# dpfried/action-segmentation

Hardware: AMD Instinct MI355X
Metric: frames/sec semi-Markov decode, CrossTask T~10k K~20 L=1024, 1/2/4/8 GPUs (higher is better)
Workload: dtype f64

## Files before the change

### action-segmentation_amd/csrc/smm_api.hip

```cpp
#include <algorithm>
#include <atomic>
#include <functional>
#include <cstdio>
#include <cstdlib>
#include <cstring>
#include <numeric>
#include <vector>
#include <unordered_map>
#include <mutex>
#include <utility>
#include <string>

#include "../../include/smmdp.h"
#include "smm_device.h"
#include "smm_launch.h"
#include "smm_plan_feedback.h"

static thread_local int g_last_hip = 0;

namespace {
struct SmmEnv {
    int spec = 1;
    int no_split = 0;
    double split_min_us = 100.0, split_ns = 0.0;
    int split_margin = 400;
    int plan_cache = 1;
    int small_wg = 1;
    int plan_feedback = 1;
    int chunk = 1;
    int chunk_p = 0;
    int chunk_lmin = 0;
    int chunk_wc = 512;
    int no_bt_window = 0;
    int fit_grid = 0;
    int verbose = 0;
#ifdef SMM_DEV
    int debug_flags = 0;
    int split_debug = 0;
    int upload_memcpy = 0;
    int emission_v2 = 0;
#endif
    std::string key;
};
std::atomic<const SmmEnv *> g_env{nullptr};
std::once_flag g_env_once;

void env_read()
{
    SmmEnv e;
    struct Item { const char *name; int *i; double *d; };
    const Item items[] = {
        {"SMM_SPEC", &e.spec, nullptr}, {"SMM_NO_SPLIT", &e.no_split, nullptr}, {"SMM_SPLIT_MIN_US", nullptr, &e.split_min_us},
        {"SMM_SPLIT_NS", nullptr, &e.split_ns}, {"SMM_SPLIT_MARGIN", &e.split_margin, nullptr},
        {"SMM_PLAN_CACHE", &e.plan_cache, nullptr}, {"SMM_SMALL_WG", &e.small_wg, nullptr}, {"SMM_PLAN_FEEDBACK", &e.plan_feedback, nullptr}, {"SMM_CHUNK", &e.chunk, nullptr}, {"SMM_CHUNK_P", &e.chunk_p, nullptr},
        {"SMM_CHUNK_WC", &e.chunk_wc, nullptr}, {"SMM_CHUNK_LMIN", &e.chunk_lmin, nullptr}, {"SMM_NO_BT_WINDOW", &e.no_bt_window, nullptr},
        {"SMM_FIT_GRID", &e.fit_grid, nullptr}, {"SMM_VERBOSE", &e.verbose, nullptr},
#ifdef SMM_DEV
        {"SMM_DEBUG_FLAGS", &e.debug_flags, nullptr}, {"SMM_SPLIT_DEBUG", &e.split_debug, nullptr},
        {"SMM_UPLOAD_MEMCPY", &e.upload_memcpy, nullptr}, {"SMM_EMISSION_V2", &e.emission_v2, nullptr},
#endif
    };
    for (const Item &it : items) {
        const char *v = std::getenv(it.name);
        if (!v) continue;
        if (it.i) *it.i = (*v == 0) ? 1 : std::atoi(v);
        if (it.d) *it.d = std::atof(v);
        e.key += it.name; e.key += '='; e.key += v; e.key += ';';
    }
    g_env.store(new SmmEnv(e), std::memory_order_release);
}
const SmmEnv &env()
{
    std::call_once(g_env_once, env_read);
    return *g_env.load(std::memory_order_acquire);
}
}

extern "C" void smm_env_reload(void)
{
    (void)env();
    env_read();
}
int smm_env_fit_grid() { return env().fit_grid; }
int smm_env_emission_v2()
{
#ifdef SMM_DEV
    return env().emission_v2;
#else
    return 0;
#endif
}

#define SMM_HIP(call)                                                         \
    do {                                                                      \
        hipError_t e_ = (call);                                               \
        if (e_ != hipSuccess) { g_last_hip = (int)e_; return SMM_ERR_HIP; }   \
    } while (0)

extern "C" const char *smm_strerror(int status)
{
    switch (status) {
    case SMM_OK: return "ok";
    case SMM_ERR_ARG: return "invalid argument";
    case SMM_ERR_UNSUPPORTED: return "shape not supported by the compiled kernels";
    case SMM_ERR_WORKSPACE: return "workspace too small";
    case SMM_ERR_HIP: return "HIP runtime error";
    case SMM_ERR_NO_DEVICE: return "no gfx950 device";
    default: return "unknown smm_status";
    }
}

extern "C" int smm_last_hip_error(void) { return g_last_hip; }
extern "C" const char *smm_version(void) { return "smmdp 0.1 (gfx950)"; }

extern "C" int smm_device_count(void)
{
    int n = 0;
    if (hipGetDeviceCount(&n) != hipSuccess) return 0;
    return n;
}

struct SmmMetaChunk { uint32_t w[512]; };

__global__ void __launch_bounds__(512) smm_meta_upload_kernel(SmmMetaChunk c, uint32_t *dst, int n)
{
    typedef const __attribute__((address_space(4))) uint32_t *smm_kernarg_ptr;
    (void)c;
#if defined(__HIP_DEVICE_COMPILE__)
    smm_kernarg_ptr ka = (smm_kernarg_ptr)__builtin_amdgcn_kernarg_segment_ptr();
    if ((int)threadIdx.x < n) dst[threadIdx.x] = ka[threadIdx.x];
#else
    (void)dst; (void)n;
#endif
}

int smm_upload_meta(void *dst_dev, const void *src_host, size_t bytes, hipStream_t stream)
{
#ifdef SMM_DEV
    if (env().upload_memcpy) return (int)hipMemcpyAsync(dst_dev, src_host, bytes, hipMemcpyHostToDevice, stream);
#endif
    const size_t words = (bytes + 3) / 4;
    const unsigned char *src = static_cast<const unsigned char *>(src_host);
    for (size_t off = 0; off < words; off += 512) {
        SmmMetaChunk c;
        const size_t n = std::min<size_t>(512, words - off);
        const size_t nb = std::min<size_t>(n * 4, bytes - off * 4);
        std::memset(&c, 0, sizeof(c));
        std::memcpy(c.w, src + off * 4, nb);
        hipLaunchKernelGGL(smm_meta_upload_kernel, dim3(1), dim3(512), 0, stream, c, static_cast<uint32_t *>(dst_dev) + off, (int)n);
    }
    return (int)hipGetLastError();
}

__global__ void __launch_bounds__(256) smm_zero_kernel(uint32_t *p, size_t nwords)
{
    const size_t head = ((16 - (reinterpret_cast<uintptr_t>(p) & 15)) & 15) >> 2;
    const size_t h = head < nwords ? head : nwords;
    const size_t nq = (nwords - h) >> 2;
    uint4 *q = reinterpret_cast<uint4 *>(p + h);
    const size_t tid = (size_t)blockIdx.x * 256 + threadIdx.x, nth = (size_t)gridDim.x * 256;
    for (size_t i = tid; i < nq; i += nth) q[i] = make_uint4(0, 0, 0, 0);
    if (tid < h) p[tid] = 0;
    const size_t tail0 = h + 4 * nq;
    if (tid < nwords - tail0) p[tail0 + tid] = 0;
}

struct SmmZeroRegions { uint32_t *p[8]; size_t nwords[8]; };
__global__ void __launch_bounds__(256) smm_zero_multi_kernel(SmmZeroRegions r)
{
    uint32_t *p = r.p[blockIdx.y];
    const size_t nwords = r.nwords[blockIdx.y];
    const size_t head = ((16 - (reinterpret_cast<uintptr_t>(p) & 15)) & 15) >> 2;
    const size_t h = head < nwords ? head : nwords;
    const size_t nq = (nwords - h) >> 2;
    uint4 *q = reinterpret_cast<uint4 *>(p + h);
    const size_t tid = (size_t)blockIdx.x * 256 + threadIdx.x, nth = (size_t)gridDim.x * 256;
    for (size_t i = tid; i < nq; i += nth) q[i] = make_uint4(0, 0, 0, 0);
    if (tid < h) p[tid] = 0;
    const size_t tail0 = h + 4 * nq;
    if (tid < nwords - tail0) p[tail0 + tid] = 0;
}

int smm_zero_multi_async(void *const *dst_dev, const size_t *bytes, int n, hipStream_t stream)
{
    SmmZeroRegions r{};
    int m = 0;
    size_t most = 0;
    for (int i = 0; i < n; ++i) {
        if (bytes[i] == 0) continue;
        if (m == 8 || (bytes[i] & 3) || (reinterpret_cast<uintptr_t>(dst_dev[i]) & 3)) {
            const int rc = smm_zero_async(dst_dev[i], bytes[i], stream);
            if (rc != (int)hipSuccess) return rc;
            continue;
        }
        r.p[m] = static_cast<uint32_t *>(dst_dev[i]);
        r.nwords[m] = bytes[i] >> 2;
        most = r.nwords[m] > most ? r.nwords[m] : most;
        ++m;
    }
    if (m == 0) return (int)hipSuccess;
    size_t blocks = (most / 4 + 255) / 256;
    blocks = blocks < 1 ? 1 : (blocks > 2048 ? 2048 : blocks);
    hipLaunchKernelGGL(smm_zero_multi_kernel, dim3((unsigned)blocks, (unsigned)m), dim3(256), 0, stream, r);
    return (int)hipGetLastError();
}

int smm_zero_async(void *dst_dev, size_t bytes, hipStream_t stream)
{
// ... 852 lines not shown
{
    int r = 1;
    while (64 * r < kp_max) r *= 2;
    return r;
}

struct Tables {
    const double *elp, *trans, *init, *len, *endpen, *logz;
};

static SmmDpArgs dp_args(const smm_shape *s, const Staged &st, const Tables &t)
{
    SmmDpArgs a{};
    a.videos = st.videos; a.order = st.order; a.n_states = st.n_states;
    a.elp = t.elp; a.trans = t.trans; a.init = t.init; a.len = t.len; a.endpen = t.endpen;
    a.hist = st.hist; a.err = st.err;
    a.c_max = s->c_max; a.k_rows = s->k_rows; a.t_max = s->t_max; a.b = s->b;
    if (s->flags & SMM_SHAPE_NO_EOS) { a.flags |= 8; a.endpen = nullptr; }
    return a;
}

static SmmPostHead post_head(const smm_shape *s, const Staged &st)
{
    return {st.videos, st.n_states, st.err, s->c_max, s->k_rows, s->b, (s->flags & SMM_SHAPE_NO_EOS) ? 1 : 0};
}
static SmmPostSide post_side(int no_eos, const double *hist, const Tables &t)
{
    return {hist, t.elp, t.trans, t.init, t.len, no_eos ? nullptr : t.endpen, t.logz};
}

struct ReversedTabs {
    double *trans_t;
    double *logz_b;
};
static ReversedTabs reversed_tabs(const smm_shape *s, double *tabs)
{
    return {tabs, tabs + (size_t)s->n_groups * s->c_max * s->c_max};
}

static int run_reversed(const smm_shape *shape, const Staged &st, double *hist, double *tabs, const Tables &t, hipStream_t hs)
{
    if (shape->flags & SMM_SHAPE_LOGZ_BOTH) return SMM_OK;
    const ReversedTabs rt = reversed_tabs(shape, tabs);
    smm_launch_transpose(t.trans, rt.trans_t, shape->n_groups, shape->c_max, hs);
    SmmDpArgs a = dp_args(shape, st, t);
    a.trans = rt.trans_t;
    a.hist = hist;
    a.flags |= 2;
    return smm_launch_logz(a, rt.logz_b, ring_regs(st.kp_max), st.c_need, hs);
}

static int run_emission(const smm_shape *s, const Staged &st, const float *x, const double *w, const double *cst,
                        const double *inv_var, const float *cons, double *elp64, float *elp32, hipStream_t stream,
                        int first = 0, int count = -1)
{
    if (!x || !w || !cst || !inv_var || s->d < 1 || (!elp64 && !elp32)) return SMM_ERR_ARG;
    if (smm_emission_lds_bytes(s->d, st.c_need) > 160 * 1024)
        return SMM_ERR_UNSUPPORTED;
    SmmEmArgs a{st.videos, st.order, st.n_states, x, w, cst, inv_var, cons, elp64, elp32, s->d, s->c_max, s->b};
    if (count < 0) smm_launch_emission(a, st.c_need, st.em_tpw, st.em_blocks, st.em_cum, s->total_frames, stream);
    else smm_launch_emission(a, st.c_need, st.em_tpw, st.em_cum_host[first + count] - st.em_cum_host[first], st.em_cum,
                             s->total_frames, stream, st.em_cum_host[first], first, count);
    SMM_HIP(hipGetLastError());
    return SMM_OK;
}

namespace {
struct DpTiming {
    std::mutex mu;
    bool on = false;
    std::vector<std::pair<hipEvent_t, hipEvent_t>> rec, pool;
    std::vector<int> tag;
} g_dp_timing;

bool dp_timing_begin(hipStream_t stream, std::pair<hipEvent_t, hipEvent_t> &ev)
{
    std::lock_guard<std::mutex> lock(g_dp_timing.mu);
    if (!g_dp_timing.on) return false;
    if (!g_dp_timing.pool.empty()) { ev = g_dp_timing.pool.back(); g_dp_timing.pool.pop_back(); }
    else if (hipEventCreate(&ev.first) != hipSuccess || hipEventCreate(&ev.second) != hipSuccess) return false;
    return hipEventRecord(ev.first, stream) == hipSuccess;
}

void dp_timing_end(hipStream_t stream, const std::pair<hipEvent_t, hipEvent_t> &ev, int tag)
{
    (void)hipEventRecord(ev.second, stream);
    std::lock_guard<std::mutex> lock(g_dp_timing.mu);
    g_dp_timing.rec.push_back(ev);
    g_dp_timing.tag.push_back(tag);
}
}

extern "C" void smm_dp_timing_enable(int on)
{
    std::lock_guard<std::mutex> lock(g_dp_timing.mu);
    g_dp_timing.on = on != 0;
}

extern "C" int smm_dp_timing_read_tagged(float *ms, int32_t *tags, int cap)
{
    std::vector<std::pair<hipEvent_t, hipEvent_t>> rec;
    std::vector<int> tag;
    {
        std::lock_guard<std::mutex> lock(g_dp_timing.mu);
        rec.swap(g_dp_timing.rec);
        tag.swap(g_dp_timing.tag);
    }
    int n = 0;
    for (auto &ev : rec) {
        float t = 0.f;
        if (hipEventSynchronize(ev.second) == hipSuccess && hipEventElapsedTime(&t, ev.first, ev.second) == hipSuccess && n < cap) {
            if (ms) ms[n] = t;
            if (tags) tags[n] = tag[n];
        }
        ++n;
    }
    std::lock_guard<std::mutex> lock(g_dp_timing.mu);
    for (auto &ev : rec) g_dp_timing.pool.push_back(ev);
    return n;
}

extern "C" int smm_dp_timing_read(float *ms, int cap) { return smm_dp_timing_read_tagged(ms, nullptr, cap); }

namespace {
hipStream_t aux_stream_n(int dev, int which);
bool aux_events_get(int dev, std::pair<hipEvent_t, hipEvent_t> &ev);
void aux_events_put(int dev, const std::pair<hipEvent_t, hipEvent_t> &ev);
}

static int run_viterbi(const smm_shape *s, const Staged &st, const double *elp, const double *trans, const double *init,
                       const double *len_scores, const double *endpen, const int64_t *class_map, int64_t *spans,
                       int64_t *labels, double *best, int32_t *n_segs, hipStream_t stream, int first = 0, int count = -1,
                       bool prep = true, bool launch = true, int timing_tag = 0)
{
    if (!elp || !trans || !init || !len_scores) return SMM_ERR_ARG;
    SmmDpArgs a = dp_args(s, st, Tables{elp, trans, init, len_scores, endpen, nullptr});
    a.class_map = class_map;
    a.spans = spans; a.labels = labels; a.best = best; a.n_segs = n_segs;
    a.stamps = st.stamps;
    if (count >= 0) { a.order = st.order + first; a.b = count; }
    const bool with_units = st.n_cv > 0 && (count < 0 || first == 0);
    if (st.n_cv > 0) {
        a.videos = st.uvideos;
        a.b_videos = s->b;
        a.chunk_anchor = st.anchors;
        if (count < 0) { a.order = st.uorder; a.b = st.n_units; }
        else if (first == 0) { a.order = st.uorder; a.b = st.u_part1; }
        else { a.order = st.uorder + st.u_part1; a.b = st.n_units - st.u_part1; }
    }
#ifdef SMM_DEV
    a.flags |= env().debug_flags;
#endif
    if (!env().spec) a.flags |= 256;
    if (st.band_mode) {
        double *len_t = st.band, *band_tab = st.band + (size_t)s->n_groups * s->c_max * SMM_BAND_ROW;
        double *dmin_t = band_tab + (size_t)s->n_groups * s->c_max * SMM_BAND_TAB;
        if (prep) smm_launch_band_tables(len_scores, st.n_states, len_t, band_tab, dmin_t, s->n_groups, s->c_max, s->k_rows, stream);
        a.len_t = len_t;
        a.band_tab = band_tab;
        a.dmin_t = dmin_t;
        a.flags |= 128;
    }
    if (ring_regs(st.kp_max) == 1 && !env().no_bt_window) {
        int w = (int)(48 * 1024 / (24 * (size_t)st.c_need)) & ~7;
        w = std::min(512, std::max(w, (2 * st.kp_max + 7) & ~7));
        const size_t bytes = sizeof(double) * ((size_t)3 * w + st.c_need + st.kp_max) * st.c_need;
        if (bytes <= 126 * 1024) { a.bt_window = w; a.bt_dyn_bytes = (int32_t)bytes; }
    }
    if (!launch) { SMM_HIP(hipGetLastError()); return SMM_OK; }
    if (with_units) smm_launch_cum_anchors(a, st.cvs, st.n_cv, st.anchors, stream);
    const int lo = (int)(a.order - (st.n_cv > 0 ? st.uorder : st.order));
    int n_small = (st.small_count > 0 && lo <= st.small_first && lo + a.b == st.small_first + st.small_count) ? st.small_count : 0;
    hipStream_t side = nullptr;
    std::pair<hipEvent_t, hipEvent_t> fj{nullptr, nullptr};
    int dev = 0;
    if (n_small > 0) {
        hipStreamCaptureStatus cap = hipStreamCaptureStatusNone;
        if (hipGetDevice(&dev) == hipSuccess && dev >= 0 && dev < 64 && hipStreamIsCapturing(stream, &cap) == hipSuccess &&
            cap == hipStreamCaptureStatusNone)
            side = aux_stream_n(dev, 1);
        if (side && !aux_events_get(dev, fj)) side = nullptr;
        if (!side) n_small = 0;
    }
    int rc_small = SMM_OK;
    if (n_small > 0) {
        SmmDpArgs as = a;
        as.order = a.order + (a.b - n_small);
        as.b = n_small;
        a.b -= n_small;
        if (hipEventRecord(fj.first, stream) != hipSuccess || hipStreamWaitEvent(side, fj.first, 0) != hipSuccess) rc_small = SMM_ERR_HIP;
        if (rc_small == SMM_OK) {
            std::pair<hipEvent_t, hipEvent_t> tev2;
            const bool timed2 = dp_timing_begin(side, tev2);
            rc_small = smm_launch_viterbi_small(as, side);
            if (timed2) dp_timing_end(side, tev2, 3);
        }
    }
    std::pair<hipEvent_t, hipEvent_t> tev;
    int rc = SMM_OK;
    if (a.b > 0) {
        const bool timed = dp_timing_begin(stream, tev);
        rc = smm_launch_viterbi(a, st.band_mode ? 16 : ring_regs(st.kp_max), st.c_need, stream);
        if (timed) dp_timing_end(stream, tev, timing_tag);
    }
    if (side) {
        if (hipEventRecord(fj.second, side) != hipSuccess || hipStreamWaitEvent(stream, fj.second, 0) != hipSuccess) rc_small = SMM_ERR_HIP;
        aux_events_put(dev, fj);
    }
    if (rc != SMM_OK) return rc;
    if (rc_small != SMM_OK) return rc_small;
    if (with_units) {
        smm_launch_chunk_stitch(a, st.cvs, st.n_cv, st.redo, stream);
        SmmDpArgs ar = a;
        ar.order = st.porder;
        ar.b = st.n_cv;
        ar.redo = st.redo;
        const int rc2 = st.band_mode ? smm_launch_viterbi_repair(ar, st.c_need, stream)
                                     : smm_launch_viterbi(ar, ring_regs(st.kp_max), st.c_need, stream);
        if (rc2 != SMM_OK) return rc2;
    }
    SMM_HIP(hipGetLastError());
    return SMM_OK;
}

extern "C" int smm_emission_f64(const smm_shape *shape, const int64_t *lengths_host, const int64_t *frame_offset_host,
                                const int32_t *group_host, const int32_t *n_states_host, const float *x, const double *w,
                                const double *cst, const double *inv_var, const float *cons, double *elp64, float *elp32,
                                void *workspace, size_t workspace_bytes, void *stream)
{
    Staged st;
    hipStream_t hs = static_cast<hipStream_t>(stream);
    int rc = stage(shape, lengths_host, frame_offset_host, group_host, nullptr, n_states_host, workspace, workspace_bytes,
                   hs, &st);
    if (rc != SMM_OK) return rc;
    return run_emission(shape, st, x, w, cst, inv_var, cons, elp64, elp32, hs);
}

extern "C" int smm_emission_bwd_f64(const smm_shape *shape, const int64_t *lengths_host, const int64_t *frame_offset_host,
                                    const int32_t *group_host, const int32_t *n_states_host, const float *x,
                                    const double *g_elp, double *g_w, double *g_cst, double *g_inv_var,
                                    void *workspace, size_t workspace_bytes, void *stream)
{
    Staged st;
    hipStream_t hs = static_cast<hipStream_t>(stream);
    if (!x || !g_elp || !g_w || !g_cst || !g_inv_var || !shape || shape->d < 1) return SMM_ERR_ARG;
    int rc = stage(shape, lengths_host, frame_offset_host, group_host, nullptr, n_states_host, workspace, workspace_bytes,
                   hs, &st, false, smm_emission_bwd_chunk());
    if (rc != SMM_OK) return rc;
    const size_t g = shape->n_groups, cm = shape->c_max, d = shape->d;
    {
        void *const zp[3] = {g_w, g_cst, g_inv_var};
        const size_t zb[3] = {sizeof(double) * g * cm * d, sizeof(double) * g * cm, sizeof(double) * d};
        SMM_HIP((hipError_t)smm_zero_multi_async(zp, zb, 3, hs));
    }
    SmmEmBwdArgs a{st.videos, st.order, st.n_states, st.em_cum, x, g_elp, g_w, g_cst, g_inv_var,
                   shape->d, shape->c_max, shape->b, st.em_blocks};
    smm_launch_emission_bwd(a, st.c_need, hs);
    SMM_HIP(hipGetLastError());
    return SMM_OK;
}

extern "C" int smm_viterbi_f64(const smm_shape *shape, const int64_t *lengths_host, const int64_t *frame_offset_host,
                               const int32_t *group_host, const int32_t *kp_host, const int32_t *n_states_host,
                               const double *elp, const double *trans, const double *init, const double *len_scores,
                               const double *endpen, const int64_t *class_map, int64_t *spans, int64_t *labels,
                               double *best, int32_t *n_segs, void *workspace, size_t workspace_bytes, void *stream)
{
    Staged st;
    hipStream_t hs = static_cast<hipStream_t>(stream);
    int rc = stage(shape, lengths_host, frame_offset_host, group_host, kp_host, n_states_host, workspace, workspace_bytes,
                   hs, &st, true);
    if (rc != SMM_OK) return rc;
    return run_viterbi(shape, st, elp, trans, init, len_scores, endpen, class_map, spans, labels, best, n_segs, hs);
}

extern "C" int smm_viterbi_f32(const smm_shape *shape, const int64_t *lengths_host, const int64_t *frame_offset_host,
                               const int32_t *group_host, const int32_t *kp_host, const int32_t *n_states_host,
                               const float *elp, const float *trans, const float *init, const float *len_scores,
                               const float *endpen, const int64_t *class_map, int64_t *spans, int64_t *labels,
                               double *best, int32_t *n_segs, void *workspace, size_t workspace_bytes, void *stream)
{
    Staged st;
    hipStream_t hs = static_cast<hipStream_t>(stream);
    int rc = stage(shape, lengths_host, frame_offset_host, group_host, kp_host, n_states_host, workspace, workspace_bytes,
                   hs, &st, true);
    if (rc != SMM_OK) return rc;
    if (!elp || !trans || !init || !len_scores) return SMM_ERR_ARG;
    const size_t g = shape->n_groups, cm = shape->c_max;
    double *t64 = st.tabs, *i64 = t64 + g * cm * cm, *l64 = i64 + g * cm, *e64 = l64 + g * shape->k_rows * cm;
    smm_launch_widen(trans, t64, g * cm * cm, hs);
    smm_launch_widen(init, i64, g * cm, hs);
    smm_launch_widen(len_scores, l64, g * shape->k_rows * cm, hs);
    if (endpen) smm_launch_widen(endpen, e64, (size_t)shape->b * cm, hs);
    smm_launch_widen(elp, st.elp, (size_t)shape->total_frames * cm, hs);
    SMM_HIP(hipGetLastError());
    return run_viterbi(shape, st, st.elp, t64, i64, l64, endpen ? e64 : nullptr, class_map, spans, labels, best, n_segs, hs);
}

namespace {
struct AuxDev {
    hipStream_t stream = nullptr, stream1 = nullptr;
    std::vector<std::pair<hipEvent_t, hipEvent_t>> events;
};
std::mutex g_aux_mu;
AuxDev g_aux[64];

// ... 930 lines not shown
```

### action-segmentation_amd/csrc/smm_device.h

```cpp
#pragma once
#include <hip/hip_runtime.h>
#include <stdint.h>

#define SMM_BIG_NEG (-1e9)
#define SMM_NEG_INF (-__builtin_huge_val())
#define SMM_MAX_STATES_DEV 32
#define SMM_BAND_DELAY 112
#define SMM_BAND_LO 16
#define SMM_BAND_N 8
#define SMM_BAND_ROW 1026
#define SMM_L0_PAIRS 64
#define SMM_GH_STRIDE (SMM_MAX_STATES_DEV + 1)
#define SMM_BAND_TAB 80
#define SMM_BAND_WIT 55

struct SmmVideo {
    int64_t frame_off;
    int64_t hist_off;
    int32_t T;
    int32_t group;
    int32_t kp;
    int32_t pad;
};

#define SMM_CHUNK_MAX_UNITS 64
struct SmmChunkVideo {
    int32_t vid;
    int32_t first_unit;
    int32_t n_chunks;
    int32_t ov;
};

struct SmmDpArgs {
    const SmmVideo *videos;
    const int32_t *order;
    const int32_t *n_states;
    const double *elp;
    const double *trans;
    const double *init;
    const double *len;
    const double *endpen;
    const int64_t *class_map;
    double *hist;
    int64_t *spans;
    int64_t *labels;
    double *best;
    int32_t *n_segs;
    int32_t *err;
    int32_t c_max, k_rows, t_max, b;
    int32_t flags;
    const double *trans_t;
    double *logz_b;
    const double *len_t;
    const double *band_tab;
    const double *dmin_t;
    const int32_t *redo;
    const double *chunk_anchor;
    int32_t b_videos;
    int32_t bt_window;
    int32_t bt_dyn_bytes;
    uint64_t *stamps;
};

__host__ __device__ inline int smm_rebalanced_rank(int c)
{
    return (c >= 14 && c % 7 == 4) ? 3 : -1;
}

__device__ __forceinline__ double smm_pack(int lo, int hi) { return __hiloint2double(hi, lo); }

__device__ __forceinline__ double smm_readlane(double x, int lane)
{
    int lo = __builtin_amdgcn_readlane(__double2loint(x), lane);
    int hi = __builtin_amdgcn_readlane(__double2hiint(x), lane);
    return smm_pack(lo, hi);
}

template <int W>
__device__ __forceinline__ double smm_group_max(double x)
{
#pragma unroll
    for (int off = W / 2; off >= 1; off >>= 1) x = fmax(x, __shfl_xor(x, off));
    return x;
}

template <int W>
__device__ __forceinline__ double smm_group_sum(double x)
{
#pragma unroll
    for (int off = W / 2; off >= 1; off >>= 1) x += __shfl_xor(x, off);
    return x;
}

template <int W>
__device__ __forceinline__ int smm_group_or(int x)
{
#pragma unroll
    for (int off = W / 2; off >= 1; off >>= 1) x |= __shfl_xor(x, off);
    return x;
}

template <int CTRL, int ROW_MASK = 0xf>
__device__ __forceinline__ double smm_dpp(double x)
{
    int lo = __double2loint(x), hi = __double2hiint(x);
    lo = __builtin_amdgcn_update_dpp(lo, lo, CTRL, ROW_MASK, 0xf, false);
    hi = __builtin_amdgcn_update_dpp(hi, hi, CTRL, ROW_MASK, 0xf, false);
    return smm_pack(lo, hi);
}

#define SMM_DPP_ROW_SHR(n) (0x110 + (n))
#define SMM_DPP_ROW_SHL(n) (0x100 + (n))
#define SMM_DPP_WAVE_ROR1 0x13C
#define SMM_DPP_ROW_BCAST15 0x142
#define SMM_DPP_ROW_BCAST31 0x143

__device__ __forceinline__ double smm_wave_ror1(double x) { return smm_dpp<SMM_DPP_WAVE_ROR1>(x); }

__device__ __forceinline__ float smm_wave_ror1f(float x)
{
    return __int_as_float(__builtin_amdgcn_update_dpp(__float_as_int(x), __float_as_int(x), SMM_DPP_WAVE_ROR1, 0xf, 0xf, false));
}

__device__ __forceinline__ bool smm_nan_bits(double x)
{
    int hi = __double2hiint(x), lo = __double2loint(x);
    asm volatile("" : "+v"(hi), "+v"(lo));
    return (hi & 0x7ff00000) == 0x7ff00000 && (((hi & 0x000fffff) | lo) != 0);
}

__device__ __forceinline__ double smm_fmax(double a, double b)
{
#ifdef SMM_FMAX_BUILTIN
    return __builtin_fmax(a, b);
#else
    double r;
    asm("v_max_f64 %0, %1, %2" : "=v"(r) : "v"(a), "v"(b));
    return r;
#endif
}

__device__ __forceinline__ double smm_max_halves(double x)
{
    const int lo = __double2loint(x), hi = __double2hiint(x);
    auto a = __builtin_amdgcn_permlane32_swap(lo, lo, false, false);
    auto b = __builtin_amdgcn_permlane32_swap(hi, hi, false, false);
    return smm_fmax(smm_pack(a[0], b[0]), smm_pack(a[1], b[1]));
}

__device__ __forceinline__ float smm_sum_halvesf(float x)
{
    const int v = __float_as_int(x);
    auto a = __builtin_amdgcn_permlane32_swap(v, v, false, false);
    return __int_as_float(a[0]) + __int_as_float(a[1]);
}

__device__ __forceinline__ float smm_sum_rows16f(float x)
{
    const int v = __float_as_int(x);
    auto a = __builtin_amdgcn_permlane16_swap(v, v, false, false);
    return __int_as_float(a[0]) + __int_as_float(a[1]);
}

__device__ __forceinline__ double smm_max_rows16(double x)
{
    const int lo = __double2loint(x), hi = __double2hiint(x);
    auto a = __builtin_amdgcn_permlane16_swap(lo, lo, false, false);
    auto b = __builtin_amdgcn_permlane16_swap(hi, hi, false, false);
    return smm_fmax(smm_pack(a[0], b[0]), smm_pack(a[1], b[1]));
}

__device__ __forceinline__ unsigned smm_row_umax16(unsigned x)
{
    asm volatile("s_nop 1\n\t"
                 "v_max_u32_dpp %0, %0, %0 row_ror:1 row_mask:0xf bank_mask:0xf\n\t"
                 "s_nop 1\n\t"
                 "v_max_u32_dpp %0, %0, %0 row_ror:2 row_mask:0xf bank_mask:0xf\n\t"
                 "s_nop 1\n\t"
                 "v_max_u32_dpp %0, %0, %0 row_ror:4 row_mask:0xf bank_mask:0xf\n\t"
                 "s_nop 1\n\t"
                 "v_max_u32_dpp %0, %0, %0 row_ror:8 row_mask:0xf bank_mask:0xf\n\t"
                 "s_nop 0"
                 : "+v"(x));
    return x;
}

__device__ __forceinline__ double smm_row_max16(double x)
{
    const int hi = __double2hiint(x), lo = __double2loint(x);
    const int sgn = hi >> 31;
    const unsigned khi = (unsigned)(hi ^ (sgn | (int)0x80000000));
    const unsigned klo = (unsigned)(lo ^ sgn);
    const unsigned mhi = smm_row_umax16(khi);
    const unsigned mlo = smm_row_umax16(khi == mhi ? klo : 0u);
    const int neg = (mhi & 0x80000000u) ? 0 : -1;
    return smm_pack((int)mlo ^ neg, (int)(mhi ^ ((unsigned)neg | 0x80000000u)));
}
```

### action-segmentation_amd/csrc/smm_viterbi.hip

```cpp
#include <type_traits>
#include "smm_device.h"

#ifdef SMM_PROFILE
#define SMM_PROF_DECL unsigned long long p_busy = 0, p_wait = 0, p_t0 = __builtin_readcyclecounter(), p_ph[4] = {0, 0, 0, 0}, p_mx = 0
#define SMM_BLOCK_BARRIER()                                                        \
    do {                                                                          \
        const unsigned long long t1 = __builtin_readcyclecounter();               \
        __syncthreads();                                                          \
        const unsigned long long t2 = __builtin_readcyclecounter();               \
        p_busy += t1 - p_t0; p_wait += t2 - t1; p_t0 = t2;                        \
    } while (0)
#define SMM_LDS_BARRIER()                                                          \
    do {                                                                          \
        const unsigned long long t1 = __builtin_readcyclecounter();               \
        smm_lds_barrier();                                                        \
        const unsigned long long t2 = __builtin_readcyclecounter();               \
        p_busy += t1 - p_t0; p_wait += t2 - t1;                                   \
        if (SMM_PROFILE == 2) { if (t2 - t1 < 150) { p_mx += 1; p_ph[jj & 3] += 1; p_ph[0] += (t1 - p_t0) << 20; } } \
        else { p_ph[jj & 3] += t1 - p_t0; p_mx = (t1 - p_t0 > p_mx) ? t1 - p_t0 : p_mx; } \
        p_t0 = t2;                                                                \
    } while (0)
#define SMM_PROF_OUT()                                                            \
    if (blockIdx.x == 0 && lane == 0) {                                           \
        unsigned long long *pp = reinterpret_cast<unsigned long long *>(a.err);   \
        pp[8 + w] = p_busy; pp[24 + w] = p_wait; pp[7] = (unsigned long long)J;   \
        if (BAND) { pp[16 + w] = p_mx; for (int ph = 0; ph < 4; ++ph) pp[32 + 4 * w + ph] = p_ph[ph]; } \
    }
#else
#define SMM_PROF_DECL do { } while (0)
#define SMM_BLOCK_BARRIER() __syncthreads()
#define SMM_LDS_BARRIER() smm_lds_barrier()
#define SMM_PROF_OUT() do { } while (0)
#endif

__device__ __forceinline__ void smm_lds_barrier()
{
    asm volatile("s_waitcnt lgkmcnt(0)\n\ts_barrier" ::: "memory");
}

#ifndef SMM_B
#define SMM_B 4
#endif
#ifndef SMM_D
#define SMM_D 1
#endif
#ifndef SMM_MOVER_STATES
#define SMM_MOVER_STATES 0
#endif
#ifndef SMM_CHAIN_DUAL
#define SMM_CHAIN_DUAL 1
#endif
#ifndef SMM_ABLATE
#define SMM_ABLATE 0
#endif
#ifndef SMM_SPEC
#define SMM_SPEC 1
#endif
#ifndef SMM_PIPE0_ALWAYS
#define SMM_PIPE0_ALWAYS 0
#endif
#ifndef SMM_SPEC8
#define SMM_SPEC8 0
#endif
#ifndef SMM_DOM_SPARSE
#define SMM_DOM_SPARSE 3
#endif
#ifndef SMM_ANCHOR
#define SMM_ANCHOR 0
#endif
#ifndef SMM_BAND_ALLWIT
#define SMM_BAND_ALLWIT 1
#endif
#ifndef SMM_HQ_ALWAYS
#define SMM_HQ_ALWAYS 0
#endif
#ifndef SMM_B8_R
#define SMM_B8_R 4
#endif

__device__ __forceinline__ void smm_best3(double &v, int &k, int &c, double v2, int k2, int c2)
{
    bool take = (v2 > v) || (v2 == v && (k2 < k || (k2 == k && c2 < c)));
    if (take) { v = v2; k = k2; c = c2; }
}

__device__ __forceinline__ void smm_wave_best3(double &v, int &k, int &c)
{
#pragma unroll
    for (int off = 32; off >= 1; off >>= 1) {
        double v2 = __shfl_xor(v, off);
        int k2 = __shfl_xor(k, off);
        int c2 = __shfl_xor(c, off);
        smm_best3(v, k, c, v2, k2, c2);
    }
}

template <int R>
__device__ __forceinline__ void smm_push(double (&A)[R], double (&L)[R], double hs, int u)
{
#pragma unroll
    for (int r0 = 0; r0 < R; r0 += 4) {
        double tq[4];
#pragma unroll
        for (int q = 0; q < 4; ++q)
            if (r0 + q < R) tq[q] = hs + L[(r0 + q - u + R) % R];
#pragma unroll
        for (int q = 0; q < 4; ++q)
            if (r0 + q < R) A[r0 + q] = smm_fmax(A[r0 + q], tq[q]);
    }
    L[(2 * R - 1 - u) % R] = smm_wave_ror1(L[(2 * R - 1 - u) % R]);
}

template <int R, int B, int D, bool TRIB = false>
__device__ __forceinline__ void smm_ring_block(double (&A)[R], double (&L)[R], double &hd, const double *h_blk,
                                               double *a_blk, int j, int jj, int lane, const double &ninf)
{
    constexpr int RING = 64 * R;
    double hv[B];
#pragma unroll
    for (int i = 0; i < B; ++i) hv[i] = h_blk[i * 2 * SMM_GH_STRIDE];
    if constexpr (D == 1) {
        smm_push<R>(A, L, hd, (jj * B) % R);
#pragma unroll
        for (int i = 1; i < B; ++i) smm_push<R>(A, L, hv[i - 1], (jj * B + i) % R);
        hd = hv[B - 1];
    } else {
#pragma unroll
        for (int i = 0; i < B; ++i) smm_push<R>(A, L, hv[i], (jj * B + i) % R);
    }
    if constexpr (R % B == 0) {
        if (lane == (((j + 1) * B) & (RING - 1)) / R) {
#pragma unroll
            for (int i = 0; i < B; ++i) {
                const int r = ((jj + 1) * B + i) % R;
                a_blk[i * SMM_MAX_STATES_DEV] = A[r];
                A[r] = ninf;
            }
        }
    } else if constexpr (B % R == 0) {
        const int d = lane - (((j + 1) * B) & (RING - 1)) / R;
        if (d >= 0 && d < B / R) {
#pragma unroll
            for (int r = 0; r < R; ++r) {
                a_blk[(d * R + r) * SMM_MAX_STATES_DEV] = A[r];
                A[r] = ninf;
            }
        }
        if constexpr (TRIB) {
            if (((d + 64) & 63) >= 64 - B / R) {
#pragma unroll
                for (int r = 0; r < R; ++r) A[r] = ninf;
            }
        }
    } else {
#pragma unroll
        for (int i = 0; i < B; ++i) {
            const int r = ((jj + 1) * B + i) % R;
            if (lane == (((j + 1) * B + i) & (RING - 1)) / R) {
                a_blk[i * SMM_MAX_STATES_DEV] = A[r];
                A[r] = ninf;
            }
        }
    }
}

template <int R>
__device__ __forceinline__ void smm_ring_init_range(double (&A)[R], double (&L)[R], const double *len_col, int cm, int off,
                                                    int kmin, int kmax, bool on, int lane)
{
    constexpr int RING = 64 * R;
#pragma unroll
    for (int r = 0; r < R; ++r) {
        const int k = (lane * R + r + off) & (RING - 1);
        A[r] = SMM_NEG_INF;
        L[r] = (on && k >= kmin && k <= kmax) ? len_col[(size_t)k * cm] : SMM_NEG_INF;
    }
}

template <int R, int B, int D, bool TRIB = false>
__device__ __forceinline__ void smm_ring_init(double (&A)[R], double (&L)[R], const double *len_col, int cm, int kp,
                                              bool on, int lane)
{
    smm_ring_init_range<R>(A, L, len_col, cm, B + D, TRIB ? B + D + 1 : 2 * B + D, kp - 1, on, lane);
}

__device__ __forceinline__ double smm_ld_agent(const double *p)
{
    return __hip_atomic_load(p, __ATOMIC_RELAXED, __HIP_MEMORY_SCOPE_AGENT);
}


__device__ __forceinline__ double smm_row_bcast(double x, int n)
{
    double u;
    asm volatile("" : "=v"(u));
#define SMM_RB(k) case k: return __builtin_amdgcn_update_dpp(u, x, 0x150 + k, 0xf, 0xf, false);
    switch (n & 15) {
        SMM_RB(0) SMM_RB(1) SMM_RB(2) SMM_RB(3) SMM_RB(4) SMM_RB(5) SMM_RB(6) SMM_RB(7)
        SMM_RB(8) SMM_RB(9) SMM_RB(10) SMM_RB(11) SMM_RB(12) SMM_RB(13) SMM_RB(14)
        default: return __builtin_amdgcn_update_dpp(u, x, 0x150 + 15, 0xf, 0xf, false);
    }
#undef SMM_RB
}

__device__ __forceinline__ void smm_band_ring_load(double (&L)[2], const double *lent_row, int off, int m, int kp, int lane)
{
    const int kr0 = (lane * 2 + off) & 127;
    const int k0 = kr0 + SMM_BAND_DELAY * m;
    const double2 v = *reinterpret_cast<const double2 *>(lent_row + k0 + 1);
    L[0] = (kr0 >= SMM_BAND_LO && k0 <= kp - 1) ? v.x : SMM_NEG_INF;
    L[1] = (kr0 != 127 && kr0 + 1 >= SMM_BAND_LO && k0 + 1 <= kp - 1) ? v.y : SMM_NEG_INF;
}

template <int R, int SPW, int NW, int HF, int B, int D = SMM_D, bool BAND = false, int TAG = 0>
__global__ void __launch_bounds__(NW * 64) __attribute__((amdgpu_waves_per_eu((BAND && NW == 4) ? 2 : 1, (BAND && NW == 4) ? 2 : (NW + 3) / 4)))
smm_viterbi_kernel(SmmDpArgs a)
{
    static_assert(!BAND || (R == 16 && (NW == 8 || NW == 4) && B == 8 && D == 0),
                  "band mode: K <= 1024, 8 waves, blocks of 8 positions, the pushers push the block's own sources");
    static_assert(BAND || R < 16, "rings of 1024 slots exist in BAND mode only");
#ifndef SMM_TRI
#define SMM_TRI 1
#endif
    constexpr bool TRI = SMM_TRI && ((BAND && D == 0) || (!BAND && B == 8 && B % R == 0 && NW == 8));
    constexpr int K0 = 2 * B + D - 1;
    constexpr int NP = NW - 1;
    constexpr int UB = (R / B) > 2 ? (R / B) : 2;
// ... 808 lines not shown
    }

    if (chunk) return;
    __syncthreads();
#ifdef SMM_PROFILE
    const unsigned long long p_kern2 = __builtin_readcyclecounter();
#endif
    const bool no_eos = (a.flags & 8) != 0;
    if (w == 0) {
        double f = SMM_NEG_INF;
        const int last = no_eos ? C - 1 : C;
        if (lane <= last) {
            for (int c = 0; c < C; ++c) {
                const double wgt = (lane == C) ? (endpen ? endpen[c] : 0.0) : trans[(size_t)lane * cm + c];
                f = fmax(f, sh_gfin[c] + wgt);
            }
            if (no_eos) f = f + elp[(size_t)T * cm + lane];
            else if (lane < C) f = f + SMM_BIG_NEG;
        }
        int kk = 0, cc = (lane <= last) ? lane : 0x7fffffff;
        if (lane > last) f = SMM_NEG_INF;
        smm_wave_best3(f, kk, cc);
        if (lane == 0) {
            sh_c = cc;
            if (a.best) a.best[vid] = f;
            if (spans) spans[T] = cmap ? cmap[cc] : cc;
            if (no_eos && labels) labels[T] = cmap ? cmap[cc] : cc;
        }
    }
    __threadfence_block();
    __syncthreads();

#ifdef SMM_DEV
    if (a.flags & 1) return;
#endif
    int n = T, to = sh_c, nseg = 0, round = 0;
    if constexpr (R == 1) {
        const int W = a.bt_window;
        if (W > 0) {
            extern __shared__ __attribute__((aligned(16))) double smm_dyn[];
            double *win_g = smm_dyn, *win_c = win_g + (size_t)W * C, *win_h = win_c + (size_t)W * C;
            double *tab_t = win_h + (size_t)W * C, *tab_l = tab_t + (size_t)C * C;
            for (int e = threadIdx.x; e < C * C; e += blockDim.x) tab_t[e] = trans[(size_t)(e / C) * cm + e % C];
            for (int e = threadIdx.x; e < kp * C; e += blockDim.x) tab_l[e] = len[(size_t)(e / C) * cm + e % C];
            const int64_t gid_l = (lane <= C) ? (cmap ? cmap[lane] : (int64_t)lane) : 0;
            const int gid_lo = (int)(gid_l & 0xffffffff), gid_hi = (int)(gid_l >> 32);
            const double ep_l = (endpen && lane < C) ? endpen[lane] : 0.0;
            bool bad = false;
            while (n > 0) {
                const int n0 = (n - W + 1 > 0) ? n - W + 1 : 0, rows = n - n0 + 1;
                __syncthreads();
                for (int e = threadIdx.x; e < rows * C; e += blockDim.x) {
                    win_g[e] = hgam[(size_t)n0 * C + e];
                    win_c[e] = hcum[(size_t)n0 * C + e];
                }
                for (int e = threadIdx.x; e < rows * C; e += blockDim.x) {
                    const int c2 = e / rows, i = e % rows;
                    win_h[(size_t)i * C + c2] = hh[(size_t)c2 * (T + 1) + n0 + i];
                }
                __syncthreads();
                if (w == 0) {
                    while (n > 0 && (n0 == 0 || n - (kp - 1) >= n0)) {
                        const int kmax = (kp - 1 < n) ? kp - 1 : n;
                        const int row = n - n0;
                        double wgt = 0.0, gmv = SMM_NEG_INF, cnl = 0.0;
                        if (lane < C) {
                            cnl = win_c[(size_t)row * C + lane];
                            wgt = (to == C) ? ep_l : tab_t[(size_t)to * C + lane];
                            gmv = win_g[(size_t)row * C + lane] + wgt;
                        }
                        if (__ballot(lane < C && smm_nan_bits(gmv)) != 0) { bad = true; break; }
                        const double rmax = smm_row_max16(gmv);
                        const double best = fmax(smm_readlane(rmax, 0), smm_readlane(rmax, 16));
                        unsigned long long fmask = __ballot(lane < C && gmv == best);
                        int k = 0x7fffffff, c = 0x7fffffff;
                        while (fmask) {
                            const int f = __builtin_amdgcn_readfirstlane(__ffsll(fmask) - 1);
                            fmask &= fmask - 1;
                            const double cn = smm_readlane(cnl, f), wf = smm_readlane(wgt, f);
                            const int lim = (kmax < k - 1) ? kmax : k - 1;
                            const int kk = lane + 1;
                            bool hit = false;
                            if (kk <= lim) hit = ((cn + (win_h[(size_t)(row - kk) * C + f] + tab_l[(size_t)kk * C + f])) + wf) == best;
                            const unsigned long long m = __ballot(hit);
                            if (m) { k = __ffsll(m); c = f; }
                        }
                        if (k < 1 || k > kmax || c < 0 || c >= C) { bad = true; break; }
                        const int s0 = n - k;
                        const int64_t gid = ((int64_t)__builtin_amdgcn_readlane(gid_hi, c) << 32) |
                                            (uint32_t)__builtin_amdgcn_readlane(gid_lo, c);
                        if (labels && lane < k) labels[s0 + lane] = gid;
                        if (spans && lane == 0) spans[s0] = gid;
                        ++nseg;
                        n = s0;
                        to = c;
                    }
                    if (lane == 0) { sh_kmin[0] = (unsigned)n; sh_kmin[1] = (unsigned)to; sh_kmin[2] = bad ? 1u : 0u; }
                }
                __syncthreads();
                n = (int)sh_kmin[0];
                to = (int)sh_kmin[1];
                if (sh_kmin[2]) {
                    if (threadIdx.x == 0) atomicExch(a.err, 1);
                    break;
                }
            }
            if (a.n_segs && threadIdx.x == 0) a.n_segs[vid] = nseg + (no_eos ? 1 : 0);
            if (a.stamps && threadIdx.x == 0) a.stamps[2 * (size_t)vid + 1] = wall_clock64();
            return;
        }
    }
#ifdef SMM_PROFILE
    unsigned long long bt_a = 0, bt_b = 0, bt_c = 0, bt_t = __builtin_readcyclecounter();
#define SMM_BT_STAMP(acc) do { const unsigned long long t_ = __builtin_readcyclecounter(); acc += t_ - bt_t; bt_t = t_; } while (0)
#else
#define SMM_BT_STAMP(acc) do { } while (0)
#endif
    if (threadIdx.x == 0) { sh_kmin[0] = 0xffffffffu; sh_kmin[1] = 0xffffffffu; sh_kmin[2] = 0xffffffffu; }
    if (threadIdx.x <= (unsigned)C) {
        const int t2 = threadIdx.x;
        int bi = C - 1;
        if (t2 < C) {
            double bv = SMM_NEG_INF;
            bi = 0;
            for (int c2 = 0; c2 < C; ++c2) {
                const double v2 = trans[(size_t)t2 * cm + c2];
                if (v2 > bv) { bv = v2; bi = c2; }
            }
        } else if (endpen) {
            for (int c2 = 0; c2 < C; ++c2)
                if (endpen[c2] == 0.0) bi = c2;
        }
        sh_guess[t2] = bi;
    }
    __syncthreads();
    const double *lcol0 = nullptr;
    if constexpr (BAND) lcol0 = a.len_t + (size_t)g * cm * SMM_BAND_ROW + 1;
    int fg = 0, kmax = 0;
    double wgt = 0.0, g0 = SMM_NEG_INF, cnl = 0.0, sp_h = 0.0, sp_l = 0.0;
    auto trip = [&](int n_, int to_) {
        fg = sh_guess[to_];
        kmax = (kp - 1 < n_) ? kp - 1 : n_;
        if (lane < C) {
            g0 = hgam[(size_t)n_ * C + lane];
            cnl = hcum[(size_t)n_ * C + lane];
            wgt = (to_ == C) ? (endpen ? endpen[lane] : 0.0) : trans[(size_t)to_ * cm + lane];
        }
        const int kk0 = w * 64 + lane + 1;
        const int kc = kk0 <= kmax ? kk0 : kmax;
        sp_h = hh[(size_t)fg * (T + 1) + n_ - kc];
        sp_l = BAND ? lcol0[(size_t)fg * SMM_BAND_ROW + kc] : len[(size_t)kc * cm + fg];
    };
    const int64_t gid_l = cmap ? cmap[lane < C ? lane : C] : (int64_t)lane;
    if (n > 0) trip(n, to);
    while (n > 0) {
        const double gmv = (lane < C) ? g0 + wgt : SMM_NEG_INF;
        const bool nan_row = __ballot(lane < C && smm_nan_bits(gmv)) != 0;
        const double rmax = smm_row_max16(gmv);
        const double best = fmax(smm_readlane(rmax, 0), smm_readlane(rmax, 16));
        unsigned long long fmask = nan_row ? 0ull : __ballot(lane < C && gmv == best);
        int k = 0x7fffffff, c = 0x7fffffff;
        SMM_BT_STAMP(bt_a);
        while (fmask) {
            const int f = __builtin_amdgcn_readfirstlane(__ffsll(fmask) - 1);
            fmask &= fmask - 1;
            const double cn = smm_readlane(cnl, f);
            const double wf = smm_readlane(wgt, f);
            const double *hcol = hh + (size_t)f * (T + 1);
            const double *lcol = BAND ? lcol0 + (size_t)f * SMM_BAND_ROW : len + f;
            const int lim = (kmax < k - 1) ? kmax : k - 1;
            for (int kb = 0; kb < lim; kb += NW * 64) {
                const int kk = kb + w * 64 + lane + 1;
                bool hit = false;
                if (kb == 0 && f == fg) {
                    if (kk <= lim) hit = ((cn + (sp_h + sp_l)) + wf) == best;
                } else if (kk <= lim) hit = ((cn + (hcol[n - kk] + lcol[BAND ? (size_t)kk : (size_t)kk * cm])) + wf) == best;
                const unsigned long long m = __ballot(hit);
                const int slot = round % 3;
                if (lane == 0 && m) atomicMin(&sh_kmin[slot], (unsigned)(kb + w * 64 + __ffsll(m)));
                if (threadIdx.x == 0) sh_kmin[(round + 1) % 3] = 0xffffffffu;
                smm_lds_barrier();
                const unsigned kf = sh_kmin[slot];
                ++round;
                if (kf != 0xffffffffu) {
                    if ((int)kf < k) { k = (int)kf; c = f; }
                    break;
                }
            }
        }
        SMM_BT_STAMP(bt_b);
        if (nan_row || k < 1 || k > kmax || c < 0 || c >= C) {
            if (threadIdx.x == 0) atomicExch(a.err, 1);
            break;
        }
        const int s = n - k;
        if (lane == 0) sh_guess[to] = c;
        const int n0 = n;
        n = s;
        to = c;
        if (n > 0) trip(n, to);
        const int64_t gid = ((int64_t)__builtin_amdgcn_readlane((int)(gid_l >> 32), c) << 32) |
                            (uint32_t)__builtin_amdgcn_readlane((int)gid_l, c);
        if (labels)
            for (int f = s + threadIdx.x; f < n0; f += blockDim.x) labels[f] = gid;
        if (threadIdx.x == 0 && spans) spans[s] = gid;
        ++nseg;
        SMM_BT_STAMP(bt_c);
    }
#ifdef SMM_PROFILE
    if (blockIdx.x == 0 && threadIdx.x == 0) {
        unsigned long long *pp = reinterpret_cast<unsigned long long *>(a.err);
        pp[40] = bt_a; pp[41] = bt_b; pp[42] = bt_c; pp[43] = (unsigned long long)nseg;
        pp[44] = p_kern1 - p_kern0; pp[45] = p_kern2 - p_kern1; pp[46] = __builtin_readcyclecounter() - p_kern2;
    }
#endif
    if (a.n_segs && threadIdx.x == 0) a.n_segs[vid] = nseg + (no_eos ? 1 : 0);
    if (a.stamps && threadIdx.x == 0) a.stamps[2 * (size_t)vid + 1] = wall_clock64();
#ifdef SMM_PROFILE_END
    if (a.best && threadIdx.x == 0) a.best[vid] = (double)wall_clock64();
#endif
}

__global__ void __launch_bounds__(256) smm_band_tables_kernel(const double *len, const int32_t *n_states, double *len_t,
                                                              double *band_tab, double *dmin_t, int cm, int k_rows)
{
    __shared__ double col[SMM_BAND_ROW];
    const int g = blockIdx.x / cm, c = blockIdx.x % cm;
    const double *src = len + (size_t)g * k_rows * cm + c;
    double *dst = len_t + ((size_t)g * cm + c) * SMM_BAND_ROW;
    const bool live = c < n_states[g];
    for (int k = threadIdx.x; k < SMM_BAND_ROW; k += blockDim.x) {
        const double v = (live && k >= 1 && k - 1 < k_rows) ? src[(size_t)(k - 1) * cm] : SMM_NEG_INF;
        dst[k] = v;
        if (k >= 1) col[k - 1] = v;
    }
    if (threadIdx.x == 0) col[SMM_BAND_ROW - 1] = SMM_NEG_INF;
    __syncthreads();
    const int wv = threadIdx.x >> 6, ln = threadIdx.x & 63;
    for (int m = wv; m <= SMM_BAND_N; m += 4) {
        const int k0 = m ? SMM_BAND_LO + SMM_BAND_DELAY * m : 33, k1 = m ? 127 + SMM_BAND_DELAY * m : 174;
        double v = m ? SMM_NEG_INF : __builtin_huge_val();
        for (int k = k0 + ln; k <= k1 && k < k_rows; k += 64) {
            const double x = col[k];
            v = m ? fmax(v, x) : fmin(v, x);
        }
#pragma unroll
        for (int off = 32; off >= 1; off >>= 1) {
            const double o = __shfl_xor(v, off);
            v = m ? fmax(v, o) : fmin(v, o);
        }
        if (!live) v = SMM_NEG_INF;
        if (ln == 0) band_tab[((size_t)g * cm + c) * SMM_BAND_TAB + m] = v;
    }
    if constexpr (SMM_ANCHOR != 0) {
        const int klo = 9, khi = (k_rows - 1 < 127) ? k_rows - 1 : 127;
        double *drow = dmin_t + ((size_t)g * cm + c) * 64;
        if (threadIdx.x < 64) {
            const int q = threadIdx.x;
            double mq = __builtin_huge_val();
            for (int d = (q ? 16 * q : 1); d < 16 * q + 16; ++d) {
                double m = __builtin_huge_val();
                if (!live || khi + d > k_rows - 1) m = SMM_NEG_INF;
                else
                    for (int k = klo; k <= khi; ++k) {
                        const double lb = col[k];
                        if (lb == SMM_NEG_INF) continue;
                        m = fmin(m, col[k + d] - lb);
                    }
                mq = fmin(mq, m);
            }
            drow[q] = mq > 0.0 ? mq * (1.0 - 0x1p-49) : mq * (1.0 + 0x1p-49);
        }
    }
    for (int d = 2 + wv; d <= SMM_BAND_WIT; d += 4) {
        const int k0 = 16 * d + 1, k1 = 16 * d + 142;
        double v = __builtin_huge_val();
        for (int k = k0 + ln; k <= k1; k += 64) v = fmin(v, k < k_rows ? col[k] : SMM_NEG_INF);
#pragma unroll
        for (int off = 32; off >= 1; off >>= 1) v = fmin(v, __shfl_xor(v, off));
        if (!live) v = SMM_NEG_INF;
        if (ln == 0) band_tab[((size_t)g * cm + c) * SMM_BAND_TAB + 16 + d] = v;
    }
}

void smm_launch_band_tables(const double *len, const int32_t *n_states, double *len_t, double *band_tab, double *dmin_t,
                            int n_groups, int cm, int k_rows, hipStream_t stream)
{
    hipLaunchKernelGGL(smm_band_tables_kernel, dim3(n_groups * cm), dim3(256), 0, stream, len, n_states, len_t, band_tab, dmin_t, cm, k_rows);
}

#include <cstdlib>
#include "../../include/smmdp.h"
#include "smm_launch.h"

template <int R, int SPW, int NW>
static int launch_if(const SmmDpArgs &a, int spw, int nw, int c_need, hipStream_t stream)
{
    if (spw != SPW || nw != NW) return 0;
    constexpr int B = (R == SMM_B8_R && NW == 8) ? 8 : SMM_B;
    const size_t dyn = (R == 1 && a.bt_window > 0) ? (size_t)a.bt_dyn_bytes : 0;
    auto go = [&](auto kernel) {
        if constexpr (R == 1) {
            static bool raised[64] = {};
            int dev = 0;
            if (hipGetDevice(&dev) != hipSuccess || dev < 0 || dev >= 64) dev = 0;
            if (!raised[dev]) {
// ... 90 lines not shown
```

Baseline: 994.6 million.

## Parallelize Viterbi backtrace across waves with speculative walkers that join paths

Adds a parallel backtrace mode, on by default, for videos at least 1024 frames long. Each wave starts from an evenly spaced time boundary with a guessed state and walks predecessors into a shared-memory list. It keeps walking until its path merges with the list of the wave below. The joined segments then write labels and spans in parallel, and the serial loop finishes only whatever prefix was left unresolved. This targets the long serial backtrace over roughly 10k frames. The cost is extra speculative work, and paths that break or never join fall back to the serial walk. The kernel also now bumps an error counter with an atomic on every launch.

```diff
diff --git a/action-segmentation_amd/csrc/smm_api.hip b/action-segmentation_amd/csrc/smm_api.hip
--- a/action-segmentation_amd/csrc/smm_api.hip
+++ b/action-segmentation_amd/csrc/smm_api.hip
@@ -18,6 +18,7 @@
 
 static thread_local int g_last_hip = 0;
 
+#define SMM_BT_PAR_MIN_T_DEFAULT 1024
 namespace {
 struct SmmEnv {
     int spec = 1;
@@ -31,6 +32,8 @@
     int chunk_p = 0;
     int chunk_lmin = 0;
     int chunk_wc = 512;
+    int bt_par = 1;
+    int bt_par_min_t = SMM_BT_PAR_MIN_T_DEFAULT;
     int no_bt_window = 0;
     int fit_grid = 0;
     int verbose = 0;
@@ -54,6 +57,7 @@
         {"SMM_SPLIT_NS", nullptr, &e.split_ns}, {"SMM_SPLIT_MARGIN", &e.split_margin, nullptr},
         {"SMM_PLAN_CACHE", &e.plan_cache, nullptr}, {"SMM_SMALL_WG", &e.small_wg, nullptr}, {"SMM_PLAN_FEEDBACK", &e.plan_feedback, nullptr}, {"SMM_CHUNK", &e.chunk, nullptr}, {"SMM_CHUNK_P", &e.chunk_p, nullptr},
         {"SMM_CHUNK_WC", &e.chunk_wc, nullptr}, {"SMM_CHUNK_LMIN", &e.chunk_lmin, nullptr}, {"SMM_NO_BT_WINDOW", &e.no_bt_window, nullptr},
+        {"SMM_BT_PAR", &e.bt_par, nullptr}, {"SMM_BT_PAR_MIN_T", &e.bt_par_min_t, nullptr},
         {"SMM_FIT_GRID", &e.fit_grid, nullptr}, {"SMM_VERBOSE", &e.verbose, nullptr},
 #ifdef SMM_DEV
         {"SMM_DEBUG_FLAGS", &e.debug_flags, nullptr}, {"SMM_SPLIT_DEBUG", &e.split_debug, nullptr},
@@ -1212,6 +1216,7 @@
     a.flags |= env().debug_flags;
 #endif
     if (!env().spec) a.flags |= 256;
+    if (env().bt_par) { a.flags |= 512; a.bt_min_t = env().bt_par_min_t; }
     if (st.band_mode) {
         double *len_t = st.band, *band_tab = st.band + (size_t)s->n_groups * s->c_max * SMM_BAND_ROW;
         double *dmin_t = band_tab + (size_t)s->n_groups * s->c_max * SMM_BAND_TAB;
diff --git a/action-segmentation_amd/csrc/smm_device.h b/action-segmentation_amd/csrc/smm_device.h
--- a/action-segmentation_amd/csrc/smm_device.h
+++ b/action-segmentation_amd/csrc/smm_device.h
@@ -59,6 +59,7 @@
     int32_t b_videos;
     int32_t bt_window;
     int32_t bt_dyn_bytes;
+    int32_t bt_min_t;
     uint64_t *stamps;
 };
 
diff --git a/action-segmentation_amd/csrc/smm_viterbi.hip b/action-segmentation_amd/csrc/smm_viterbi.hip
--- a/action-segmentation_amd/csrc/smm_viterbi.hip
+++ b/action-segmentation_amd/csrc/smm_viterbi.hip
@@ -73,6 +73,12 @@
 #endif
 #ifndef SMM_HQ_ALWAYS
 #define SMM_HQ_ALWAYS 0
+#endif
+#ifndef SMM_BT_CAP
+#define SMM_BT_CAP 256
+#endif
+#ifndef SMM_BT_SPEC_ROUNDS
+#define SMM_BT_SPEC_ROUNDS 3
 #endif
 #ifndef SMM_B8_R
 #define SMM_B8_R 4
@@ -1187,6 +1193,160 @@
         sp_l = BAND ? lcol0[(size_t)fg * SMM_BAND_ROW + kc] : len[(size_t)kc * cm + fg];
     };
     const int64_t gid_l = cmap ? cmap[lane < C ? lane : C] : (int64_t)lane;
+    if ((a.flags & 512) != 0 && T >= a.bt_min_t && T < (1 << 26)) {
+        constexpr int CAP = SMM_BT_CAP, SR = SMM_BT_SPEC_ROUNDS;
+        static_assert(sizeof(sh_gh) >= (size_t)(NW / 2) * CAP * 4 && sizeof(sh_junk) >= (size_t)(NW / 2) * CAP * 4, "walker lists");
+        static_assert(sizeof(sh_e) >= (size_t)(6 * NW + 4) * 4, "walker books");
+        unsigned *const list_lo = reinterpret_cast<unsigned *>(&sh_gh[0][0][0][0]);
+        unsigned *const list_hi = reinterpret_cast<unsigned *>(&sh_junk[0][0][0][0]);
+        auto list_of = [&](int p) { return p < NW / 2 ? list_lo + p * CAP : list_hi + (p - NW / 2) * CAP; };
+        int *const bk = reinterpret_cast<int *>(&sh_e[0][0][0]);
+        enum { BT_STOPPED = 0, BT_BROKEN = 1, BT_UNJOINED = 2, BT_JOINED = 3 };
+        int gs = (lane <= C) ? sh_guess[lane] : 0;
+        auto wpred = [&](int n_, int to_, int &k_out, int &c_out) -> bool {
+            const int fg_ = __builtin_amdgcn_readlane(gs, to_);
+            const int kmax_ = (kp - 1 < n_) ? kp - 1 : n_;
+            double g_ = SMM_NEG_INF, cn_ = 0.0, w_ = 0.0, sh_[SR], sl_[SR];
+            if (lane < C) {
+                g_ = hgam[(size_t)n_ * C + lane];
+                cn_ = hcum[(size_t)n_ * C + lane];
+                w_ = (to_ == C) ? (endpen ? endpen[lane] : 0.0) : trans[(size_t)to_ * cm + lane];
+            }
+#pragma unroll
+            for (int r = 0; r < SR; ++r) {
+                const int kk0 = r * 64 + lane + 1;
+                const int kc = kk0 <= kmax_ ? kk0 : kmax_;
+                sh_[r] = hh[(size_t)fg_ * (T + 1) + n_ - kc];
+                sl_[r] = BAND ? lcol0[(size_t)fg_ * SMM_BAND_ROW + kc] : len[(size_t)kc * cm + fg_];
+            }
+            const double gmv = (lane < C) ? g_ + w_ : SMM_NEG_INF;
+            if (__ballot(lane < C && smm_nan_bits(gmv)) != 0) return false;
+            const double rmax = smm_row_max16(gmv);
+            const double best = fmax(smm_readlane(rmax, 0), smm_readlane(rmax, 16));
+            unsigned long long fmask = __ballot(lane < C && gmv == best);
+            int k = 0x7fffffff, c = 0x7fffffff;
+            while (fmask) {
+                const int f = __builtin_amdgcn_readfirstlane(__ffsll(fmask) - 1);
+                fmask &= fmask - 1;
+                const double cn = smm_readlane(cn_, f);
+                const double wf = smm_readlane(w_, f);
+                const double *hcol = hh + (size_t)f * (T + 1);
+                const double *lcol = BAND ? lcol0 + (size_t)f * SMM_BAND_ROW : len + f;
+                const int lim = (kmax_ < k - 1) ? kmax_ : k - 1;
+                int kb = 0;
+                bool found = false;
+                if (f == fg_) {
+#pragma unroll
+                    for (int r = 0; r < SR; ++r) {
+                        if (!found && r * 64 < lim) {
+                            const int kk = r * 64 + lane + 1;
+                            const bool hit = kk <= lim && ((cn + (sh_[r] + sl_[r])) + wf) == best;
+                            const unsigned long long m = __ballot(hit);
+                            if (m) { k = r * 64 + __ffsll(m); c = f; found = true; }
+                        }
+                    }
+                    kb = SR * 64;
+                }
+                for (; !found && kb < lim; kb += 64) {
+                    const int kk = kb + lane + 1;
+                    bool hit = false;
+                    if (kk <= lim) hit = ((cn + (hcol[n_ - kk] + lcol[BAND ? (size_t)kk : (size_t)kk * cm])) + wf) == best;
+                    const unsigned long long m = __ballot(hit);
+                    if (m) { k = kb + __ffsll(m); c = f; found = true; }
+                }
+            }
+            if (k < 1 || k > kmax_ || c < 0 || c >= C) return false;
+            k_out = k;
+            c_out = c;
+            return true;
+        };
+        unsigned *const mine = list_of(w);
+        const int b_lo = (w == 0) ? 0 : (int)((long long)w * T / NW);
+        int wn = (w == NW - 1) ? T : (int)((long long)(w + 1) * T / NW), wto = __builtin_amdgcn_readfirstlane((w == NW - 1) ? sh_c : C);
+        int cnt = 1, how = BT_STOPPED, join = -1;
+        if (lane == 0) mine[0] = ((unsigned)wn << 6) | (unsigned)wto;
+        auto wstep = [&]() -> bool {
+            int k2 = 0, c2 = 0;
+            if (cnt >= CAP || !wpred(wn, wto, k2, c2)) return false;
+            if (lane == wto) gs = c2;
+            wn = __builtin_amdgcn_readfirstlane(wn - k2);
+            wto = __builtin_amdgcn_readfirstlane(c2);
+            if (lane == 0) mine[cnt] = ((unsigned)wn << 6) | (unsigned)wto;
+            ++cnt;
+            return true;
+        };
+        while (wn > b_lo)
+            if (!wstep()) { how = BT_BROKEN; break; }
+        if (lane == 0) bk[w] = cnt;
+        __syncthreads();
+        SMM_BT_STAMP(bt_a);
+        if (w > 0 && how == BT_STOPPED) {
+            const unsigned *const low = list_of(w - 1);
+            const int lcnt = bk[w - 1];
+            int j = 0;
+            for (;;) {
+                const unsigned x = ((unsigned)wn << 6) | (unsigned)wto;
+                while (j < lcnt) {
+                    const unsigned v = (j + lane < lcnt) ? low[j + lane] : 0u;
+                    const unsigned long long above = __ballot(v > x);
+                    const int adv = (~above == 0ull) ? 64 : __ffsll(~above) - 1;
+                    j += adv;
+                    if (adv < 64) break;
+                }
+                if (j >= lcnt) { how = BT_UNJOINED; break; }
+                if (low[j] == x) { how = BT_JOINED; join = j; break; }
+                if (wn <= 0) { how = BT_UNJOINED; break; }
+                if (!wstep()) { how = BT_BROKEN; break; }
+            }
+        }
+        if (lane == 0) { bk[NW + w] = cnt; bk[2 * NW + w] = how; bk[3 * NW + w] = join; }
+        __syncthreads();
+        SMM_BT_STAMP(bt_b);
+        if (threadIdx.x == 0) {
+            int q = NW - 1, from = 0, total = 0;
+            for (;;) {
+                bk[4 * NW + q] = from;
+                total += bk[NW + q] - 1 - from;
+                if (q == 0 || bk[2 * NW + q] != BT_JOINED) break;
+                from = bk[3 * NW + q];
+                --q;
+            }
+            bk[6 * NW] = q;
+            bk[6 * NW + 1] = (int)list_of(q)[bk[NW + q] - 1];
+            bk[6 * NW + 2] = total;
+        }
+        __syncthreads();
+        const int q_last = bk[6 * NW];
+        for (int q = NW - 1; q >= q_last; --q) {
+            const unsigned *const lq = list_of(q);
+            const int last = bk[NW + q] - 1;
+            for (int i = bk[4 * NW + q] + w; i < last; i += NW) {
+                const unsigned hi_w = lq[i], lo_w = lq[i + 1];
+                const int n0 = (int)(hi_w >> 6), s = (int)(lo_w >> 6);
+                const int c = __builtin_amdgcn_readfirstlane((int)(lo_w & 63u));
+                const int64_t gid = ((int64_t)__builtin_amdgcn_readlane((int)(gid_l >> 32), c) << 32) |
+                                    (uint32_t)__builtin_amdgcn_readlane((int)gid_l, c);
+                if (labels)
+                    for (int f = s + lane; f < n0; f += 64) labels[f] = gid;
+                if (lane == 0 && spans) spans[s] = gid;
+            }
+        }
+        n = (int)((unsigned)bk[6 * NW + 1] >> 6);
+        to = bk[6 * NW + 1] & 63;
+        nseg = bk[6 * NW + 2];
+        if (threadIdx.x == 0) atomicAdd(a.err + 1, n == 0 ? 1 : 0x10000);
+#ifdef SMM_PROFILE
+        if (blockIdx.x == 0 && threadIdx.x == 0) {
+            unsigned long long cc = 0;
+            for (int p = 0; p < NW; ++p) {
+                const int n1 = bk[p], n2 = bk[NW + p] - bk[p];
+                cc |= (unsigned long long)((n1 < 31 ? n1 : 31) | ((n2 < 7 ? n2 : 7) << 5)) << (8 * p);
+            }
+            reinterpret_cast<unsigned long long *>(a.err)[47] = cc;
+        }
+#endif
+        SMM_BT_STAMP(bt_c);
+    }
     if (n > 0) trip(n, to);
     while (n > 0) {
         const double gmv = (lane < C) ? g0 + wgt : SMM_NEG_INF;
```

Result: faster. 1.019 billion (median of 6 runs) (+2.5%).
